# thomasdeppisch/eMagLS

Hardware: AMD Instinct MI355X
Metric: eMagLS filter sets/s (N=4, 2702 dirs, 512 taps) (higher is better)
Workload: dtype f64; 1 GPU; BASELINE config 3: getEMagLsFilters em32 r=4.2cm N=4 complex-SH, 2702 dirs, 512 taps, 48 kHz; one filter set per step, inputs resident in HBM; dirs=2702, taps=512, sim_order=19, bins=512, k_cut=43, designs_resident_per_gpu=128, designs_per_batch=32, batches_in_flight=4, distinct_hrir_sets_resident=20, parallelism=independent jobs per GPU, one RCCL gather

## Files before the change

### emagls_amd/build.py

```python
from __future__ import annotations

import argparse
import os
import subprocess
import sys
from concurrent.futures import ThreadPoolExecutor

HERE = os.path.dirname(os.path.abspath(__file__))
CSRC = os.path.join(HERE, "csrc")
OBJ = os.path.join(HERE, "build")
LIBDIR = os.path.join(HERE, "lib")
LIB = os.path.join(LIBDIR, "libemagls.so")
SOURCES = ["sh_basis.hip", "modal.hip", "fft.hip", "gram_chol.hip", "factor.hip", "gramroute.hip", "sweep.hip", "sweep_persist.hip", "sweep_synth.hip", "sweep_reg.hip", "synth_debug.hip", "factor_debug.hip", "fft_debug.hip", "gram_debug.hip", "dspace.hip", "atf.hip", "decode.hip", "decode_stream.hip", "field_stream.hip", "rotate.hip", "rotate3.hip", "resample.hip", "render.hip", "render_api.hip", "response.hip", "response_api.hip", "array_irs.hip", "shoebox.hip", "array_irs_api.hip", "emash.hip", "wide.hip", "wide_array.hip", "microbench.hip",
           "switches.hip", "decode_api.hip", "field_api.hip", "host_pools.hip", "plan_setup.hip", "plan_run.hip", "batch_run.hip", "capi.hip", "jobs.hip"]
HIPCC = os.environ.get("HIPCC", "/opt/rocm/bin/hipcc")
FLAGS = ["--offload-arch=gfx950", "-O3", "-std=c++17", "-fPIC", "-ffp-contract=off", "-Wall", "-Wno-unused-function",
         "-Wno-unused-result", "-Wno-unused-value"]


def _newest_header():
    hs = [os.path.join(CSRC, f) for f in os.listdir(CSRC) if f.endswith(".hpp")]
    hs.append(os.path.join(os.path.dirname(HERE), "include", "emagls.h"))
    return max(os.path.getmtime(h) for h in hs)


def _compile(src, force):
    obj = os.path.join(OBJ, src.replace(".hip", ".o"))
    srcp = os.path.join(CSRC, src)
# ... 38 lines not shown
```

### emagls_amd/csrc/batch_run.hip

```cpp
#include "host_internal.hpp"

void emagls_batch_forget(emagls_batch* b, emagls_plan* p) {
    for (auto& q : b->plans) if (q == p) q = nullptr;
}

namespace {
void batch_sweep_stage(emagls_batch& b) {
    const int nb = (int)b.plans.size();
    std::vector<HalfSweepArgs> ha((size_t)nb);
    for (int j = 0; j < nb; ++j) ha[j] = emagls_half_args(*b.plans[j]);
    if (b.atf_share || b.geo_share)
        for (int j = 1; j < nb; ++j) {
            ha[j].G = ha[0].G; ha[j].Yri = ha[0].Yri; ha[j].Mw = ha[0].Mw; ha[j].cond_ok = ha[0].cond_ok;
            ha[j].bsc = ha[0].bsc; ha[j].smap = ha[0].smap;
            ha[j].skip_flag = ha[0].skip_flag;
        }
    const bool reg = b.plans[0]->sweep_persist && reg_sweep_wanted(b.plans.data(), nb);
    for (auto* q : b.plans) q->reg_sweep = reg;
    if (!reg && nb > SWEEP_MULTI_MAX) throw Error(EMAGLS_ERR_UNSUPPORTED, "internal: more than 16 designs in a batch need the register-resident sweep");
    HalfSweepMulti h{};
    h.n = std::min(nb, SWEEP_MULTI_MAX);
    for (int j = 0; j < h.n; ++j) h.a[j] = ha[j];
    emagls_plan& q0 = *b.plans[0];
    const int kk0 = std::max(q0.kcut0, 1);
// ... 102 lines not shown
    HIP_CHECK(hipStreamSynchronize(b.stream));
    HIP_CHECK(hipMemsetAsync(b.cmp_flag.get(), 0, 16, b.stream));
    emagls_plan& p0 = *b.plans[0];
    for (size_t j = 1; j < b.plans.size(); ++j)
        for (const char* name : names) launch_compare_words(p0.get(name), b.plans[j]->get(name), p0.bufs[name].bytes, b.cmp_flag.get<int>(), b.stream);
    int differ = 0;
    HIP_CHECK(hipMemcpyAsync(&differ, b.cmp_flag.get(), sizeof differ, hipMemcpyDeviceToHost, b.stream));
    HIP_CHECK(hipStreamSynchronize(b.stream));
    checked_version = ver;
    return same = differ == 0;
}
void batch_set_sharing(emagls_batch& b, bool& field, bool share) {
    if (share == field) return;
    for (auto* p : b.plans) drop_plan_graphs(*p);
    drop_batch_graphs(b);
    if (&field == &b.geo_share) batch_geo_forget(b);
    field = share;
}
void batch_run_two_graphs(emagls_batch& b, CapturedGraph& pre, void (*stage)(emagls_batch&, int), int pre_part, int launches) {
    const bool replay = b.use_graph && b.eager_runs >= 1;
    if (replay && !pre) pre.capture(b.stream, [&] { stage(b, pre_part); });
    if (replay && !b.post) b.post.capture(b.stream, [&] { stage(b, 2); });
    b.used = 0;
    if (replay) pre.launch(b.stream); else stage(b, pre_part);
    batch_sweep_stage(b);
    if (replay) b.post.launch(b.stream); else stage(b, 2);
    mark_executed(b, launches);
    if (!replay) ++b.eager_runs;
}
template <typename Pre> void batch_run_per_plan(emagls_batch& b, bool replay, Pre pre, void (*post)(emagls_plan&), int launches) {
    emagls_plan& p0 = *b.plans[0];
// ... 52 lines not shown
    for (auto* p : b.plans)
        if (!p->have_hrirs || !p->have_hrir_grid || !p->have_atfs)
            throw Error(EMAGLS_ERR_ARG, "every plan of the batch needs its HRIRs, its grid and the ATFs");
    batch_atf_decide_sharing(b);
    emagls_plan& p0 = *b.plans[0];
    if (b.atf_share && p0.sweep_persist) { batch_run_two_graphs(b, b.group[0], batch_atf_shared_stage, 0, 1); return; }
    batch_run_per_plan(b, b.use_graph && b.eager_runs >= 1,
                       [&](emagls_plan& p) { if (b.atf_share && &p != &p0) from_atf_subject_pre_stage(p); else plan_pre_stage(p); },
                       from_atf_post_sweep, sweep_launch_count(p0));
}

uint64_t batch_geo_version(const emagls_batch& b) {
    uint64_t ver = 0;
    for (const emagls_plan* p : b.plans) ver = (ver * 1000003ull + p->atf_side_version) * 1000003ull + p->solo_runs;
    return ver;
}
void batch_geo_decide_sharing(emagls_batch& b) {
    bool share = false;
    if (b.geo_want && b.plans.size() > 1) {
        emagls_plan& p0 = *b.plans[0];
        bool eligible = (p0.d.kind == EMAGLS_KIND_EMAGLS || p0.d.kind == EMAGLS_KIND_EMAGLS2 || p0.d.kind == EMAGLS_KIND_EMA_CH) && !p0.wide &&
                        !p0.diffuse && !p0.custom_basis;
        for (auto* p : b.plans) {
            const emagls_design_desc &x = p->d, &y = p0.d;
            eligible = eligible && x.kind == y.kind && x.order == y.order && x.fs == y.fs && x.len == y.len && x.nsamp == y.nsamp &&
                       x.ndirs == y.ndirs && x.mic_radius == y.mic_radius && x.nmics == y.nmics && x.basis == y.basis &&
                       x.sim_order_pad == y.sim_order_pad && p->wide == p0.wide && p->diffuse == p0.diffuse && p->custom_basis == p0.custom_basis &&
                       p->real_internal == p0.real_internal && p->gram_from == p0.gram_from && p->hh_end == p0.hh_end && p->n_h == p0.n_h &&
                       p->g0 == p0.g0 && p->sweep_persist == p0.sweep_persist;
        }
        share = eligible && batch_inputs_same(b, {"hrir_azi", "hrir_zen", "mic_azi", "mic_zen"}, b.geo_checked_version, b.geo_inputs_same);
    }
    batch_set_sharing(b, b.geo_share, share);
}
void geo_hrir_side(emagls_plan& h, emagls_plan& g, emagls_plan& p0, hipStream_t st) {
    subject_reset(h, st);
    h.sync_used = 0;
    hrir_spectra(h, p0, st);
    if (g.hh_end > 1) {
        hrir_hh_rows(h, g, st);
        hrir_hh_back(hh_factor_args(h, g, nullptr, g.get<double>("cond_ok")), g, st);
    }
    hrir_gram_ls_rows(h, g, p0, true, st);
    if (p0.synth) launch_synth_winit(h.get("W"), p0.get("Pm"), p0.C, (int)p0.d.nmics, std::max(p0.kcut0, 1), p0.P, h.get("Winit"), st, true);
}
void batch_geo_stage(emagls_batch& b, int part) {
    emagls_plan& p0 = *b.plans[0];
    StreamLoan loan(b.plans, b.stream);
    const int n = (int)b.plans.size();
    auto hrir_side = [&](int first) {
        if (first >= n) return;
        if (b.lanes) {
            BatchScope sc(n - first, b.stride);
            geo_hrir_side(*b.plans[first], *b.plans[first], p0, b.stream);
        } else {
            for (int j = first; j < n; ++j) geo_hrir_side(*b.plans[j], p0, p0, b.stream);
        }
    };
    if (part == 1) {
        hrir_side(0);
    } else if (part == 0) {
        plan_pre_stage(p0);
        if (b.lanes && n > 1) {
            emagls_plan& g = p0;
            const bool cb = g.cplx_basis;
            const int gf = g.gram_from, hh_end = g.hh_end, ldSh = g.ldS_h;
            const int ls_end = std::min(g.kcut0, g.P);
            const size_t g_stride_b = sizeof(cplx) * (size_t)g.C * g.ldD;
            auto bc = [&](const char* name, size_t off, size_t bytes) {
                if (!g.has(name) || bytes == 0) return;
                bytes = std::min(bytes, g.bufs[name].bytes - off);
                launch_broadcast_lanes(g.get<char>(name) + off, bytes, b.stride, n - 1, b.stream);
            };
            if (hh_end > 1) {
                bc("Yc", 0, g.bufs["Yc"].bytes);
                bc(cb ? "R" : "Rc", 0, g.bufs[cb ? "R" : "Rc"].bytes);
                bc("Vws", 0, sizeof(cplx) * (size_t)(hh_end - 1) * g.C * ldSh);
                bc("Nw", 0, sizeof(cplx) * (size_t)(hh_end - 1) * g.C * g.C);
                bc("tauw", 0, sizeof(double) * (size_t)(hh_end - 1) * g.C);
                bc("cond_ok", 0, sizeof(double) * (size_t)g.P);
            }
            if (gf > 0 && gf < ls_end) {
                bc("G", (size_t)(gf - g.g0) * g_stride_b, (size_t)(ls_end - gf) * g_stride_b);
                bc("Mw", 0, sizeof(cplx) * (size_t)ls_end * g.C * g.C);
            }
        }
        hrir_side(1);
    } else if (b.lanes) {
        BatchScope sc(n, b.stride);
        Scoped from(p0.geo_from, &p0);
        emagls_post_sweep(p0);
    } else {
        for (auto* p : b.plans) {
            Scoped from(p->geo_from, &p0);
            emagls_post_sweep(*p);
        }
    }
}
void batch_execute_geo(emagls_batch& b) {
    const bool warm = batch_geo_next_is_warm(b);
    if (!warm) {
        b.geo_kept_version = ~0ull;
        b.geo_ran_version = batch_geo_version(b);
        b.geo_cold_pending = true;
    }
    batch_run_two_graphs(b, warm ? b.warm : b.group[0], batch_geo_stage, warm ? 1 : 0, sweep_launch_count(*b.plans[0]));
    b.last_form = warm ? 2 : 1;
    ++(warm ? b.geo_warm_runs : b.geo_cold_runs);
}

void batch_magls_decide_sharing(emagls_batch& b, bool sweep_needed) {
    bool share = false;
    emagls_plan& p0 = *b.plans[0];
    if (b.geo_want && b.plans.size() > 1 && !p0.custom_basis && !p0.diffuse && (p0.sweep_persist || !sweep_needed)) {
        share = batch_inputs_same(b, {"hrir_azi", "hrir_zen"}, b.geo_checked_version, b.geo_inputs_same);
        for (auto* p : b.plans) share = share && !p->custom_basis && p->d.fs == p0.d.fs;
    }
    batch_set_sharing(b, b.geo_share, share);
}
// ... 286 lines not shown
```

### emagls_amd/csrc/capi.hip

```cpp
#include "host_internal.hpp"

namespace {

struct CachedPlan {
    std::unique_ptr<emagls_plan> plan;
    emagls_design_desc desc{};
    int device = 0;
    bool busy = false;
    uint64_t last_use = 0;
};
std::mutex g_cache_mu;
std::vector<CachedPlan> g_cache;
uint64_t g_cache_tick = 0;

int one_shot(const emagls_design_desc& desc, const double* hL, const double* hR, const double* azi, const double* zen,
             const double* mic_azi, const double* mic_zen, const double* atf, const double* atf_azi, const double* atf_zen,
             void* wL, void* wR, double* mean_dev, const void* Y_hrir = nullptr, const void* Y_mic = nullptr) {
    return guarded([&] {
        int dev = 0;
        HIP_CHECK(hipGetDevice(&dev));
        emagls_plan* p = nullptr;
        std::unique_ptr<emagls_plan> fresh;
        bool cached = false;
        {
// ... 424 lines not shown
            for (int i = 0; i < p->sweep_launches && 2 * (size_t)i + 1 < p->sweep_events.size(); ++i) {
                float t = 0.f;
                HIP_CHECK(hipEventElapsedTime(&t, p->sweep_events[2 * i], p->sweep_events[2 * i + 1]));
                tot += t;
                ++n;
            }
        }
        *total_ms = tot;
        *launches = n;
    });
}
int emagls_plan_debug_buffer(emagls_plan* p, const char* name, void* dst, size_t* nbytes) {
    return guarded([&] {
        DeviceGuard dg(p ? p->device : -1);
        if (!p || !name || !nbytes) throw Error(EMAGLS_ERR_ARG, "null pointer");
        auto it = p->bufs.find(name);
        if (it == p->bufs.end()) throw Error(EMAGLS_ERR_ARG, std::string("unknown buffer ") + name);
        if (!dst) { *nbytes = it->second.bytes; return; }
        HIP_CHECK(hipStreamSynchronize(p->stream));
        const size_t n = std::min(*nbytes, it->second.bytes);
        HIP_CHECK(hipMemcpy(dst, it->second.p, n, hipMemcpyDeviceToHost));
        *nbytes = n;
    });
}
void* emagls_plan_stream(emagls_plan* p) { return p ? (void*)p->stream : nullptr; }

int emagls_batch_create(emagls_plan** plans, int nplans, emagls_batch** batch) {
    return guarded([&] {
        if (!plans || !batch || nplans < 1) throw Error(EMAGLS_ERR_ARG, "invalid argument");
        const int batch_max = std::max(g_batch_max.load(), g_batch_max_override);
// ... 387 lines not shown
```

### emagls_amd/csrc/dspace.hip

```cpp
#include "kernels.hpp"

namespace emagls {

constexpr double COND_LIMIT = 1.0e4;

template <typename T, int QT_TD>
__global__ void __launch_bounds__(512) qt_kernel(const T* __restrict__ Yc, int64_t ldY, const T* __restrict__ E, int ldE,
                                                 int D, int S, int C, int nOrders, T* __restrict__ QT, int64_t ldD, size_t bstride) {
    Yc = boff(Yc, bstride); E = boff(E, bstride); QT = boff(QT, bstride);
    extern __shared__ __attribute__((aligned(16))) char dyn[];
    T* ys = reinterpret_cast<T*>(dyn);
    const int ldq = S + 1;
    const int d0 = blockIdx.x * QT_TD;
    for (int idx = threadIdx.x; idx < QT_TD * S; idx += blockDim.x) {
        const int dl = idx / S, s = idx % S;
        ys[(size_t)dl * ldq + s] = (d0 + dl < D) ? Yc[(int64_t)(d0 + dl) * ldY + s] : zero_of<T>();
    }
    __syncthreads();
    const int dl = threadIdx.x % QT_TD;
    const T* y = ys + (size_t)dl * ldq;
    for (int c = threadIdx.x / QT_TD; c < C; c += 512 / QT_TD) {
        const T* e = E + (int64_t)c * ldE;
        for (int n = 0; n < nOrders; ++n) {
            const int sb = n * n, se = min(S, (n + 1) * (n + 1));
// ... 150 lines not shown
__global__ void cond_flag_kernel(const double* __restrict__ sv, int C, int P, int hh_end, double* __restrict__ cond_ok, size_t bstride) {
    sv = boff(sv, bstride); cond_ok = boff(cond_ok, bstride);
    const int kb = blockIdx.x * blockDim.x + threadIdx.x;
    if (kb >= P) return;
    double smax = 0.0, smin = INFINITY;
    for (int i = 0; i < C; ++i) { const double s = sv[(int64_t)kb * C + i]; smax = fmax(smax, s); smin = fmin(smin, s); }
    cond_ok[kb] = (kb >= hh_end || smax <= COND_LIMIT * smin) ? 1.0 : 0.0;
}

template <typename T>
__global__ void __launch_bounds__(256) yri_accurate_kernel(const T* __restrict__ Q, int64_t ldQ, const cplx* __restrict__ Z,
                                                           int ldS, const double* __restrict__ cond_ok, int D, int S, int C, int k0,
                                                           cplx* __restrict__ Yri, int64_t ldD, size_t bstride) {
    Q = boff(Q, bstride); Z = boff(Z, bstride); cond_ok = boff(cond_ok, bstride); Yri = boff(Yri, bstride);
    const int kb = k0 + blockIdx.y;
    if (cond_ok[kb] != 0.0) return;
    const int c = threadIdx.x >> 3, dl = threadIdx.x & 7;
    if (c >= C) return;
    for (int d = blockIdx.x * 8 + dl; d < D; d += gridDim.x * 8) {
        const T* q = Q + (int64_t)d * ldQ;
        const cplx* z = Z + ((int64_t)kb * C + c) * ldS;
        cplx a0 = mk(0, 0), a1 = mk(0, 0);
        int s = 0;
        for (; s + 1 < S; s += 2) { cfma(a0, conj(q[s]), z[s]); cfma(a1, conj(q[s + 1]), z[s + 1]); }
        if (s < S) cfma(a0, conj(q[s]), z[s]);
        Yri[((int64_t)(kb - k0) * C + c) * ldD + d] = a0 + a1;
    }
}

constexpr int YA_SCH = 32;
__global__ void __launch_bounds__(256) yri_accurate_cm_kernel(const double* __restrict__ Ycm, int64_t ldY, const cplx* __restrict__ Z, int ldS,
                                                              const double* __restrict__ cond_ok, int D, int S, int C, int k0,
                                                              cplx* __restrict__ Yri, int64_t ldD, size_t bstride) {
    Ycm = boff(Ycm, bstride); Z = boff(Z, bstride); cond_ok = boff(cond_ok, bstride); Yri = boff(Yri, bstride);
    const int kb = k0 + blockIdx.y;
    if (cond_ok[kb] != 0.0) return;
    __shared__ __attribute__((aligned(16))) cplx zs[32][YA_SCH + 1];
    const int tid = threadIdx.x, wave = tid >> 6, lane = tid & 63;
    const int d = blockIdx.x * 128 + (wave & 1) * 64 + lane;
    const int ch0 = (wave >> 1) * 16;
    const int dc = d < D ? d : D - 1;
    cplx acc[16];
#pragma unroll
    for (int i = 0; i < 16; ++i) acc[i] = mk(0, 0);
    for (int s0 = 0; s0 < S; s0 += YA_SCH) {
        __syncthreads();
        for (int idx = tid; idx < 32 * YA_SCH; idx += 256) {
            const int c = idx / YA_SCH, s = idx % YA_SCH;
            zs[c][s] = (c < C && s0 + s < S) ? Z[((int64_t)kb * C + c) * ldS + s0 + s] : mk(0, 0);
        }
        __syncthreads();
// ... 108 lines not shown
```

### emagls_amd/csrc/gram_chol.hip

```cpp
#include <cstdlib>
#include <vector>

#include "device_mem.hpp"

namespace emagls {

typedef double double4_t __attribute__((ext_vector_type(4)));
typedef double double2_t __attribute__((ext_vector_type(2)));

template <typename T> struct GramAcc;
template <> struct GramAcc<double> {
    double4_t r[2][2];
    __device__ void init() { for (int a = 0; a < 2; ++a) for (int b = 0; b < 2; ++b) r[a][b] = double4_t{0, 0, 0, 0}; }
};
template <> struct GramAcc<cplx> {
    double4_t r[2][2], i[2][2];
    __device__ void init() {
        for (int a = 0; a < 2; ++a) for (int b = 0; b < 2; ++b) { r[a][b] = double4_t{0, 0, 0, 0}; i[a][b] = double4_t{0, 0, 0, 0}; }
    }
};

__device__ __forceinline__ void gram_step(GramAcc<double>& acc, const double (&a)[2], const double (&b)[2]) {
#pragma unroll
    for (int x = 0; x < 2; ++x)
// ... 572 lines not shown
            KERNEL_CHECK();
            chol_update_kernel<T><<<bgrid(nbt * (nbt + 1) / 2), 256, 0, st>>>((T*)G, S, j0, nbt, batch_ctx().stride);
            KERNEL_CHECK();
        }
    }
}
void launch_cholesky(void* G, int S, bool is_cplx, int* flag, hipStream_t st) {
    if (is_cplx) chol_impl<cplx>(G, S, flag, st); else chol_impl<double>(G, S, flag, st);
}

__global__ void __launch_bounds__(256) zsolve_flagged_kernel(cplx* __restrict__ Z, int ldS, const cplx* __restrict__ R,
                                                             const cplx* __restrict__ Rinv, const double* __restrict__ cond_ok,
                                                             int S, int C, int k0, size_t bstride) {
    Z = boff(Z, bstride); R = boff(R, bstride); Rinv = boff(Rinv, bstride); cond_ok = boff(cond_ok, bstride);
    const int kb = k0 + blockIdx.x;
    if (cond_ok[kb] != 0.0) return;
    __shared__ cplx as[32][33];
    __shared__ cplx ri[32][33];
    const int c = threadIdx.x >> 3, part = threadIdx.x & 7;
    cplx* z = Z + ((int64_t)kb * C + (c < C ? c : 0)) * ldS;
    const int nblk = (S + NB - 1) / NB;
    for (int J = nblk - 1; J >= 0; --J) {
        const int j0 = J * NB;
        for (int idx = threadIdx.x; idx < NB * NB; idx += 256) ri[idx / NB][idx % NB] = Rinv[(int64_t)J * NB * NB + idx];
        for (int m = 0; m < 4; ++m) {
            const int jj = part + 8 * m, j = j0 + jj;
            cplx acc = mk(0, 0);
            if (c < C && j < S) {
                acc = z[j];
                const cplx* rrow = R + (int64_t)j * S;
                for (int i = j0 + NB; i < S; ++i) { cplx p = mk(0, 0); cfma(p, z[i], conj(rrow[i])); acc = acc - p; }
// ... 119 lines not shown
```

### emagls_amd/csrc/host_internal.hpp

```cpp
#pragma once
#include <atomic>
#include <chrono>
#include <cstdlib>
#include <cstring>
#include <deque>
#include <map>
#include <memory>
#include <mutex>
#include <shared_mutex>
#include <string>
#include <thread>
#include <utility>
#include <vector>

#include "../../include/emagls.h"
#include "array_model.hpp"
#include "device_mem.hpp"
#include "kernels.hpp"

using namespace emagls;

struct emagls_batch;
void emagls_batch_forget(emagls_batch* b, emagls_plan* p);

// ... 326 lines not shown
    bool lanes = false;
    size_t stride = 0;
    hipStream_t stream = nullptr;
    bool own_stream = true;
    bool atf = false, atf_share = false, atf_inputs_same = false;
    uint64_t atf_checked_version = ~0ull;
    bool magls = false;
    bool geo_want = false, geo_share = false, geo_inputs_same = false;
    uint64_t geo_checked_version = ~0ull;
    uint64_t geo_kept_version = ~0ull;
    uint64_t geo_ran_version = ~0ull;
    bool geo_cold_pending = false;
    CapturedGraph warm;
    int last_form = 0;
    long long geo_cold_runs = 0, geo_warm_runs = 0;
    emagls::DevMem cmp_flag;
    int nstreams = 1;
    hipStream_t side[3] = {nullptr, nullptr, nullptr};
    CapturedGraph group[4];
    int prof_level = 0;
    hipEvent_t sweep_ev[2] = {nullptr, nullptr};
    CapturedGraph post;
    bool side0_external = false;
    int order_hint = 0;
    int groups = 1;
    CapturedGraph group_hh[4];
    hipStream_t hh_stream[4] = {nullptr, nullptr, nullptr, nullptr};
    bool defer_hh = false;
    bool alone = true;
    int eager_runs = 0;
// ... 47 lines not shown

constexpr double GRAM_COND_EST = 3.0e3;

inline bool forks_streams(const emagls_plan& p) { return p.nstreams >= 2; }

extern thread_local hipStream_t g_plan_stream_shared;
void plan_routes(emagls_plan& p);
void synth_pairing(const double* azi, const double* zen, int M, int* smap);
void plan_alloc_routes(emagls_plan& p);
void plan_setup(emagls_plan& p);

void stage_prologue(emagls_plan& p, int mode, const int64_t* didx, int64_t Dh);
void execute_ls(emagls_plan& p);
void magls_post_sweep(emagls_plan& p);
bool plan_defers_hh_route(const emagls_plan& p);
void hrir_spectra(emagls_plan& h, const emagls_plan& g, hipStream_t st);
FactorArgs hh_factor_args(emagls_plan& h, emagls_plan& g, int* sweeps_out, double* cond_ok);
void hrir_hh_rows(emagls_plan& h, emagls_plan& g, hipStream_t st);
void hrir_hh_back(const FactorArgs& fa, const emagls_plan& g, hipStream_t st);
void hrir_gram_ls_rows(emagls_plan& h, emagls_plan& g, const emagls_plan& src, bool lanes_share, hipStream_t st);
void subject_reset(emagls_plan& p, hipStream_t st);
void emagls_pre_sweep(emagls_plan& p);
HalfSweepArgs emagls_half_args(emagls_plan& p);
struct SweepGate {
    struct Entry { hipEvent_t ev; int slots; };
    struct State { std::deque<Entry> inflight; std::vector<hipEvent_t> pool; int capacity = 0; };
    static std::mutex& mutex();
    static State& state();
    std::unique_lock<std::mutex> lock;
    hipStream_t st;
    int slots;
// ... 30 lines not shown
```

### emagls_amd/csrc/kernels.hpp

```cpp
#pragma once
#include <algorithm>
#include <functional>

#include "common.hpp"

namespace emagls {

void launch_zero(void* p, size_t bytes, hipStream_t st);
void launch_compare_words(const void* a, const void* b, size_t bytes, int* differ, hipStream_t st);
void launch_broadcast_lanes(const void* src, size_t bytes, size_t stride, int nlanes, hipStream_t st);
struct LanePtrs { void* p[64]; };
void launch_scatter_lanes(const void* srcL, const void* srcR, size_t stride, size_t bytes, int n, const LanePtrs& dst, hipStream_t st);
void launch_gather_buffers(const LanePtrs& src, const LanePtrs& dst, int nbuf, size_t bytes, hipStream_t st);
struct BufferMoves { const void* src[96]; void* dst[96]; size_t bytes[96]; int n; };
void launch_move_buffers(const BufferMoves& m, hipStream_t st);
void launch_ch_basis(int N, int M, const double* azi, bool cplx_basis, void* out, int ld, hipStream_t st, bool out_real = false);
void launch_sh_coeff(int N, double* tab, hipStream_t st);
inline size_t esz(bool c) { return c ? sizeof(cplx) : sizeof(double); }
inline size_t sh_coeff_count(int N) { return (size_t)2 * (N + 1) * (N + 1) + 2 * (N + 1); }
void launch_sh_basis(int N, int64_t D, const double* azi, const double* zen, const double* tab, bool cplx_basis,
                     void* Y, int64_t ld, hipStream_t st);
void launch_transpose_conj(const void* Y, int64_t D, int64_t S, int64_t ldY, void* Yt, int64_t Dpad, int64_t ldYt,
                           bool is_cplx, bool conj_it, hipStream_t st);

// ... 65 lines not shown
int persist_sweep_dpw(int D);
int sweep_cu_budget();
bool persist_sweep_fits(int D, int C, int ndesigns);
bool synth_sweep_fits(int D, int nmics, int nOrd, int ndesigns);
bool synth_sweep_supported(int D, int nmics, int nOrd);
int synth_nord_pad(int nOrd);
void launch_synth_prepare(const void* bn, int nOrd, int P, void* bsc, const void* Zlo, int ldZ, int nOut, int M, const int* smap, double* Pm, hipStream_t st);
void launch_synth_mt(const void* Mw, const double* Pm, int nOut, int M, int k0, int P, const void* W, void* Mt, void* Winit, hipStream_t st);
void launch_synth_winit(const void* W, const void* Pm, int nOut, int M, int k0, int P, void* Winit, hipStream_t st, bool shared_geometry);
void launch_synth_rows(const void* U, int nchunks, const void* Pm, const void* Mw, int nOut, int M, int k_lo, int k_hi, int P, void* W, hipStream_t st,
                       bool shared_geometry = false);
int synth_ls_chunks(int D);
void launch_synth_ls(const void* Hc, int64_t ldH, int n_c, const void* bsc, int nord_pad, const double* dir_azi, const double* dir_zen, const double* mic_azi,
                     const double* mic_zen, const int* smap, int D, int M, int P, int kb_lo, int kb_hi, void* Upart, hipStream_t st, bool shared_geometry = false);
void launch_sweep_synth(const HalfSweepMulti& m, hipStream_t st);
void synth_cosines_debug(const double* dir_azi, const double* dir_zen, int64_t ndirs, const double* mic_azi, const double* mic_zen, int nmics, double* x2);
void synth_operand_debug(const void* bsc, int nbins, int nord_pad, const double* x, int64_t nx, int gs, void* g_plus, void* g_minus);
int reg_sweep_max_units();
bool reg_sweep_supported(int D, int nmics, int nunits, int nOrd);
size_t reg_sweep_ll_bytes(int D, int nmics);
int reg_sweep_capacity(int D);
int reg_sweep_slots_per_xcd();
int reg_sweep_pick_waves(int D, int ndesigns);
int reg_sweep_gate_cost(int D, int ndesigns);
bool reg_sweep_fits(int D, int nmics, int nunits, int nOrd, int ndesigns);
void launch_sweep_reg(const HalfSweepArgs* args_dev, const HalfSweepArgs& a0, int n, hipStream_t st);
double reg_contract_selftest();
double gram_tile_selftest(bool four);
void store_sweep_args(const HalfSweepArgs* host, int n, HalfSweepArgs* dev, hipStream_t st);
void launch_sweep_finalize(const void* Wpart, void* W, int nWG, int C, int P, int kb_last, hipStream_t st);
// ... 205 lines not shown
```

### emagls_amd/csrc/plan_run.hip

```cpp
#include "host_internal.hpp"

namespace {
void stage_hrir_basis(emagls_plan& p) {
    hipStream_t st = p.stream;
    const bool cb = p.cplx_basis;
    if (p.d.kind == EMAGLS_KIND_MAGLS_2D) {
        launch_ch_basis(p.d.order, (int)p.D, p.get<double>("hrir_azi"), cb, p.get("Ycm"), (int)p.ldD, st, !cb);
    } else if (!p.custom_basis) {
        launch_sh_coeff(p.simOrder, p.get<double>("sh_tab"), st);
        launch_sh_basis(p.simOrder, p.D, p.get<double>("hrir_azi"), p.get<double>("hrir_zen"), p.get<double>("sh_tab"), cb,
                        p.get("Ycm"), p.ldD, st);
    }
    launch_transpose_conj(p.get("Ycm"), p.D, p.S, p.ldD, p.get("Yc"), p.Dpad, p.ldS, cb, true, st);
    p.mark("sh_basis");
    launch_gram(p.get("Yc"), p.D, p.S, p.ldS, cb, p.get("Gp"), nullptr, p.get("R"), p.S, st);
    p.mark("gram_mfma");
    launch_cholesky(p.get("R"), p.S, cb, p.get<int>("flag"), st);
    p.mark("cholesky");
    if (p.wide) return;
    launch_qform(p.get("Yc"), p.get("R"), p.get("Rinv"), p.S, p.D, p.ldS, cb, p.get("Q"), st);
    p.mark("qform");
}

void record_sweep_event(emagls_plan& p, size_t i) {
// ... 487 lines not shown
void magls_post_sweep(emagls_plan& p) {
    hipStream_t st = p.stream;
    const bool cb = p.cplx_basis;
    if (p.diffuse)
        launch_diffuse_constraint(p.get("W"), p.get("Xc"), cb, 0, 1, p.get("Hfull"), (int)p.D, p.C, p.ldD, p.P, st);
    launch_filter_epilogue(p.get("W"), p.C, p.nfft, (int)p.d.len, p.get("tw"), p.get<double>("grpd"),
                           cb ? (p.d.kind == EMAGLS_KIND_MAGLS_2D ? 2 : 1) : 0, 0, 0,
                           p.out_cplx ? 1 : 0, p.get("wL"), p.get("wR"), st);
    p.mark("epilogue");
}

bool plan_defers_hh_route(const emagls_plan& p) {
    const int k0 = std::max(p.kcut0, 1);
    return sw_int<Sw::DEFER_HH>() != 0 && p.synth && !p.diffuse && p.prof_level == 0 && p.d.kind != EMAGLS_KIND_EMA_SH && p.gram_from > 0 && p.hh_end > 1 && p.hh_end <= k0 - 1;
}
void hrir_spectra(emagls_plan& h, const emagls_plan& g, hipStream_t st) {
    const emagls_design_desc& d = h.d;
    const int ls_end = std::min(g.kcut0, g.P);
    launch_twiddles(h.nfft, h.get("tw"), st);
    launch_hrir_grpdelay(h.get<double>("hL"), h.get<double>("hR"), d.nsamp, d.ndirs, h.nfft, h.get("tw"), h.get<double>("dirsum"),
                         h.get<double>("grpd"), st);
    launch_hrir_fft(h.get<double>("hL"), h.get<double>("hR"), d.nsamp, h.D, nullptr, h.nfft, h.get("tw"), h.get<double>("grpd"), 0, ls_end,
                    h.kcut0, h.get("Hc"), h.get<double>("Habs"), h.ldD, st, ls_end > 0 ? h.get<double>("HcT") : nullptr,
                    round_up(4 * std::max(ls_end, 1), 64));
}
FactorArgs hh_factor_args(emagls_plan& h, emagls_plan& g, int* sweeps_out, double* cond_ok) {
    const int ls_end = std::min(g.kcut0, g.P);
    FactorArgs fa{};
    fa.S = g.S_h; fa.C = g.C; fa.ldS = g.ldS_h; fa.kb0 = 1; fa.P = g.P;
    fa.Tn = g.get("Tn"); fa.bn = g.get<cplx>("bn"); fa.nOrders = g.n_h + 1; fa.bn_stride = g.simOrder + 1;
    fa.reg_mode = 0; fa.reg_c = SVD_REGUL_CONST;
    fa.Z = h.get<cplx>("Z");
    fa.Mw = g.get<cplx>("Mw");
    fa.Vws = g.get<cplx>("Vws"); fa.sv = g.get<double>("sv");
    fa.Hq = h.get<cplx>("Hq"); fa.ldHq = g.ldS_h; fa.hq_estride = (int64_t)ls_end * g.ldS_h; fa.ls_end = std::min(ls_end, g.hh_end);
    fa.hq_conj = 1;
    fa.route = g.get<int>("route"); fa.status = h.get<int>("flag");
    fa.cond_limit = 10.0 * GRAM_COND_EST;
// ... 453 lines not shown
```

### emagls_amd/csrc/switches.hpp

```cpp
#pragma once
#include <climits>
#include <cmath>

namespace emagls {

#define EMAGLS_SWITCHES(X) \
    X(PLAN_CACHE,        INT,  4,     0, INT_MAX,   PROCESS, "shapes the one-shot entry points keep alive (0 = off)") \
    X(BATCH_MAX,         INT,  8,     1, 32,        PROCESS, "initial limit of designs per batch, read at load time (emagls_set_batch_max changes it at run time; the job scheduler sets it per chunk)") \
    X(BATCH_GROUPS,      INT,  2,     1, 4,         CALL,    "lane groups of a batch of more than 8 designs before its sweep (1 = one launch sequence)") \
    X(BATCH_LANES,       ON0,  1,     0, 1,         CALL,    "=0: batches in stream mode (per-plan pipelines) instead of lane mode") \
    X(DEBUG_LANES,       ON1,  0,     0, 1,         CALL,    "=1: why a batch was refused lane mode or common routes, on stderr") \
    X(STAGGER,           ON0,  1,     0, 1,         PROCESS, "=0: both lane groups of a batch issue the stages before the sweep in one order (default: complementary orders)") \
    X(DEFER_HH,          INT,  1,     0, 2,         PROCESS, "the orthonormal route of the low bins next to the sweep: 0 never, 1 batches and designs that have the device to themselves, 2 every lane batch") \
    X(GEO_KEEP,          ON0,  1,     0, 1,         PROCESS, "=0: sharing batches run their geometry stages on every execute") \
    X(GRAM_LDS,          ON0,  1,     0, 1,         PROCESS, "=0: lane batches take the K-split Gram kernel + reduce instead of the LDS-staged one") \
    X(GRAM_MFMA4,        ON1,  0,     0, 1,         CALL,    "=1: the Gram tile on the 4 x 4 x 4 MFMA shape (measured slower; the tests' second form)") \
    X(XCD_RUNS,          ON0,  1,     0, 1,         PROCESS, "=0: gram_lds, gemm_tn_f64, synth_ls take their tiles in dispatch order instead of XCD-aware runs") \
    X(GRAM_ROUTE,        ON0,  1,     0, 1,         CALL,    "=0: no Gram route (all bins Householder + Jacobi)") \
    X(GRAM_COND_EST,     REAL, 3e3,   -HUGE_VAL, HUGE_VAL, CALL, "conditioning estimate below which the Gram route starts (the device check stays at 3e4)") \
    X(JACOBI_RUN,        INT,  0,     1, INT_MAX,   PROCESS, "bins per Jacobi workgroup on the Gram route (0: single bins where the stages are forked, runs of 2 in lane groups)") \
    X(REAL_INTERNAL,     ON0,  1,     0, 1,         CALL,    "=0: complex-basis eMagLS / eMagLS2 designs on the complex-arithmetic pipeline") \
    X(NO_GRAPH,          ON1,  0,     0, 1,         CALL,    "=1: eager launches instead of hipGraph replay (plans and batches, when they are created)") \
    X(STREAMS,           INT,  0,     1, 4,         CALL,    "streams of a single plan (0: one, until emagls_plan_set_streams)") \
    X(ONESHOT_STREAMS,   INT,  1,     1, 3,         CALL,    "streams of the one-shot plans of array designs") \
    X(SWEEP_PERSIST,     ON0,  1,     0, 1,         CALL,    "=0: launch-per-bin sweep instead of the persistent one") \
    X(PERSIST_GLOBAL,    ON1,  0,     0, 1,         CALL,    "=1: write-through granules even when a design sits on one XCD") \
    X(SWEEP_SYNTH,       ON0,  1,     0, 1,         CALL,    "=0: array designs on materialised operands instead of the synthesising sweep (when a plan is created)") \
    X(SWEEP_TWIN,        ON0,  1,     0, 1,         CALL,    "=0: launches of 9-16 designs as two independent workgroups per CU instead of twin workgroups") \
    X(SWEEP_REG,         INT,  1,     0, 2,         CALL,    "register-resident sweep: 0 never (the slab form), 1 for launches of more than 8 designs, 2 always") \
// ... 56 lines not shown
```

Measured before the change: 3919 filter sets/s.

## Share one least-squares operand per bin across geometry-sharing HRIR batches

When every plan in a batch shares the array and HRIR geometry, the per-bin Y_reg_inv least-squares operand is computed once for the batch. That covers the Householder/Z-solve bins and the Gram bins through a new synthesis kernel. Each HRIR set then needs only its spectra plus a small Hc·Yls row product kernel, instead of carrying its own LS rows through the factor chain. The batch keeps extra device buffers and invalidates its graphs whenever they reallocate. It also adds a switch, on by default, to turn the path off.

After: 4309 filter sets/s, median of 6. 1.1x the previous value.

```diff
diff --git a/emagls_amd/build.py b/emagls_amd/build.py
--- a/emagls_amd/build.py
+++ b/emagls_amd/build.py
@@ -11,7 +11,7 @@
 OBJ = os.path.join(HERE, "build")
 LIBDIR = os.path.join(HERE, "lib")
 LIB = os.path.join(LIBDIR, "libemagls.so")
-SOURCES = ["sh_basis.hip", "modal.hip", "fft.hip", "gram_chol.hip", "factor.hip", "gramroute.hip", "sweep.hip", "sweep_persist.hip", "sweep_synth.hip", "sweep_reg.hip", "synth_debug.hip", "factor_debug.hip", "fft_debug.hip", "gram_debug.hip", "dspace.hip", "atf.hip", "decode.hip", "decode_stream.hip", "field_stream.hip", "rotate.hip", "rotate3.hip", "resample.hip", "render.hip", "render_api.hip", "response.hip", "response_api.hip", "array_irs.hip", "shoebox.hip", "array_irs_api.hip", "emash.hip", "wide.hip", "wide_array.hip", "microbench.hip",
+SOURCES = ["sh_basis.hip", "modal.hip", "fft.hip", "gram_chol.hip", "factor.hip", "gramroute.hip", "sweep.hip", "sweep_persist.hip", "sweep_synth.hip", "sweep_reg.hip", "ls_shared.hip", "synth_debug.hip", "factor_debug.hip", "fft_debug.hip", "gram_debug.hip", "dspace.hip", "atf.hip", "decode.hip", "decode_stream.hip", "field_stream.hip", "rotate.hip", "rotate3.hip", "resample.hip", "render.hip", "render_api.hip", "response.hip", "response_api.hip", "array_irs.hip", "shoebox.hip", "array_irs_api.hip", "emash.hip", "wide.hip", "wide_array.hip", "microbench.hip",
            "switches.hip", "decode_api.hip", "field_api.hip", "host_pools.hip", "plan_setup.hip", "plan_run.hip", "batch_run.hip", "capi.hip", "jobs.hip"]
 HIPCC = os.environ.get("HIPCC", "/opt/rocm/bin/hipcc")
 FLAGS = ["--offload-arch=gfx950", "-O3", "-std=c++17", "-fPIC", "-ffp-contract=off", "-Wall", "-Wno-unused-function",
diff --git a/emagls_amd/csrc/batch_run.hip b/emagls_amd/csrc/batch_run.hip
--- a/emagls_amd/csrc/batch_run.hip
+++ b/emagls_amd/csrc/batch_run.hip
@@ -140,7 +140,7 @@
     if (share == field) return;
     for (auto* p : b.plans) drop_plan_graphs(*p);
     drop_batch_graphs(b);
-    if (&field == &b.geo_share) batch_geo_forget(b);
+    if (&field == &b.geo_share || &field == &b.geo_ls_shared) batch_geo_forget(b);
     field = share;
 }
 void batch_run_two_graphs(emagls_batch& b, CapturedGraph& pre, void (*stage)(emagls_batch&, int), int pre_part, int launches) {
@@ -223,6 +223,12 @@
     uint64_t ver = 0;
     for (const emagls_plan* p : b.plans) ver = (ver * 1000003ull + p->atf_side_version) * 1000003ull + p->solo_runs;
     return ver;
+}
+static bool batch_geo_ls_shared_wanted(const emagls_plan& p0) {
+    const int ls_end = std::min(p0.kcut0, p0.P);
+    const bool gram_ls = p0.gram_from > 0 && p0.gram_from < ls_end;
+    return sw_on<Sw::GEO_LS_SHARED>() && p0.d.kind != EMAGLS_KIND_EMAGLS2 && ls_end > 1 && p0.C <= 32 && (!gram_ls || p0.synth) &&
+           (p0.hh_end <= 1 || p0.has("Z"));
 }
 void batch_geo_decide_sharing(emagls_batch& b) {
     bool share = false;
@@ -241,6 +247,7 @@
         share = eligible && batch_inputs_same(b, {"hrir_azi", "hrir_zen", "mic_azi", "mic_zen"}, b.geo_checked_version, b.geo_inputs_same);
     }
     batch_set_sharing(b, b.geo_share, share);
+    batch_set_sharing(b, b.geo_ls_shared, share && batch_geo_ls_shared_wanted(*b.plans[0]));
 }
 void geo_hrir_side(emagls_plan& h, emagls_plan& g, emagls_plan& p0, hipStream_t st) {
     subject_reset(h, st);
@@ -253,17 +260,50 @@
     hrir_gram_ls_rows(h, g, p0, true, st);
     if (p0.synth) launch_synth_winit(h.get("W"), p0.get("Pm"), p0.C, (int)p0.d.nmics, std::max(p0.kcut0, 1), p0.P, h.get("Winit"), st, true);
 }
+void geo_spectra_side(emagls_plan& h, emagls_plan& p0, hipStream_t st) {
+    subject_reset(h, st);
+    h.sync_used = 0;
+    hrir_spectra(h, p0, st, false);
+}
+void geo_ls_shared_rows(emagls_plan& h, emagls_plan& p0, const void* yls, hipStream_t st) {
+    launch_ls_shared_rows(h.get("Hc"), h.ldD, std::min(p0.kcut0, p0.P), yls, p0.ldD, (int)p0.D, p0.C, p0.P, h.get("W"), st);
+    if (p0.synth) launch_synth_winit(h.get("W"), p0.get("Pm"), p0.C, (int)p0.d.nmics, std::max(p0.kcut0, 1), p0.P, h.get("Winit"), st, true);
+}
+void geo_yls_stage(emagls_batch& b, hipStream_t st) {
+    emagls_plan& g = *b.plans[0];
+    const bool cb = g.cplx_basis;
+    const int ls_end = std::min(g.kcut0, g.P), hh_ls = std::min(g.hh_end, ls_end), gf = g.gram_from;
+    cplx* yls = b.yls.get<cplx>();
+    if (hh_ls > 1) {
+        HIP_CHECK(hipMemcpyAsync(b.zls.get(), g.get("Z"), sizeof(cplx) * (size_t)hh_ls * g.C * g.ldS_h, hipMemcpyDeviceToDevice, st));
+        launch_zsolve_flagged(b.zls.get(), g.ldS_h, g.get(cb ? "R" : "Rc"), g.get(cb ? "Rinv" : "Rinvc"), nullptr, g.S_h, g.C, hh_ls, 1, st);
+        launch_yri_accurate(g.get("Yc"), g.ldS, cb, b.zls.get(), g.ldS_h, nullptr, (int)g.D, g.S_h, g.C, hh_ls, 1, yls, g.ldD, st,
+                            g.custom_basis ? nullptr : g.get("Ycm"), g.ldD);
+    }
+    if (gf > 0 && gf < ls_end)
+        launch_yls_gram(g.get("bsc"), synth_nord_pad(g.simOrder + 1), g.get<double>("hrir_azi"), g.get<double>("hrir_zen"), g.get<double>("mic_azi"),
+                        g.get<double>("mic_zen"), g.get<int>("smap"), g.get<double>("Pm"), g.get("Mw"), (int)g.D, g.C, gf, ls_end,
+                        yls, g.ldD, st);
+}
 void batch_geo_stage(emagls_batch& b, int part) {
     emagls_plan& p0 = *b.plans[0];
     StreamLoan loan(b.plans, b.stream);
     const int n = (int)b.plans.size();
-    auto hrir_side = [&](int first) {
+    auto each = [&](int first, auto f) {
         if (first >= n) return;
         if (b.lanes) {
             BatchScope sc(n - first, b.stride);
-            geo_hrir_side(*b.plans[first], *b.plans[first], p0, b.stream);
+            f(*b.plans[first], *b.plans[first]);
         } else {
-            for (int j = first; j < n; ++j) geo_hrir_side(*b.plans[j], p0, p0, b.stream);
+            for (int j = first; j < n; ++j) f(*b.plans[j], p0);
+        }
+    };
+    auto hrir_side = [&](int first) {
+        if (b.geo_ls_shared) {
+            each(first, [&](emagls_plan& h, emagls_plan&) { geo_spectra_side(h, p0, b.stream); });
+            each(0, [&](emagls_plan& h, emagls_plan&) { geo_ls_shared_rows(h, p0, b.yls.get(), b.stream); });
+        } else {
+            each(first, [&](emagls_plan& h, emagls_plan& g) { geo_hrir_side(h, g, p0, b.stream); });
         }
     };
     if (part == 1) {
@@ -294,6 +334,7 @@
                 bc("Mw", 0, sizeof(cplx) * (size_t)ls_end * g.C * g.C);
             }
         }
+        if (b.geo_ls_shared) geo_yls_stage(b, b.stream);
         hrir_side(1);
     } else if (b.lanes) {
         BatchScope sc(n, b.stride);
@@ -312,6 +353,14 @@
         b.geo_kept_version = ~0ull;
         b.geo_ran_version = batch_geo_version(b);
         b.geo_cold_pending = true;
+        if (b.geo_ls_shared) {
+            const emagls_plan& p0 = *b.plans[0];
+            const int ls_end = std::min(p0.kcut0, p0.P), hh_ls = std::min(p0.hh_end, ls_end);
+            const void *y0 = b.yls.get(), *z0 = b.zls.get();
+            b.yls.grow(sizeof(cplx) * (size_t)(ls_end - 1) * p0.C * p0.ldD);
+            b.zls.grow(sizeof(cplx) * (size_t)std::max(hh_ls, 1) * p0.C * p0.ldS_h);
+            if (b.yls.get() != y0 || b.zls.get() != z0) { b.group[0].reset(); b.warm.reset(); }
+        }
     }
     batch_run_two_graphs(b, warm ? b.warm : b.group[0], batch_geo_stage, warm ? 1 : 0, sweep_launch_count(*b.plans[0]));
     b.last_form = warm ? 2 : 1;
diff --git a/emagls_amd/csrc/capi.hip b/emagls_amd/csrc/capi.hip
--- a/emagls_amd/csrc/capi.hip
+++ b/emagls_amd/csrc/capi.hip
@@ -462,6 +462,18 @@
     return guarded([&] {
         DeviceGuard dg(p ? p->device : -1);
         if (!p || !name || !nbytes) throw Error(EMAGLS_ERR_ARG, "null pointer");
+        if (std::string(name) == "Yls") {
+            emagls_batch* b = p->owner;
+            if (!b || !b->geo_share || !b->geo_ls_shared || !b->yls.get()) throw Error(EMAGLS_ERR_ARG, "Yls: the plan's batch keeps no such operand");
+            const emagls_plan& p0 = *b->plans[0];
+            const size_t bytes = sizeof(cplx) * (size_t)(std::min(p0.kcut0, p0.P) - 1) * p0.C * p0.ldD;
+            if (!dst) { *nbytes = bytes; return; }
+            HIP_CHECK(hipStreamSynchronize(b->stream));
+            const size_t n = std::min(*nbytes, bytes);
+            HIP_CHECK(hipMemcpy(dst, b->yls.get(), n, hipMemcpyDeviceToHost));
+            *nbytes = n;
+            return;
+        }
         auto it = p->bufs.find(name);
         if (it == p->bufs.end()) throw Error(EMAGLS_ERR_ARG, std::string("unknown buffer ") + name);
         if (!dst) { *nbytes = it->second.bytes; return; }
diff --git a/emagls_amd/csrc/dspace.hip b/emagls_amd/csrc/dspace.hip
--- a/emagls_amd/csrc/dspace.hip
+++ b/emagls_amd/csrc/dspace.hip
@@ -188,7 +188,7 @@
                                                            cplx* __restrict__ Yri, int64_t ldD, size_t bstride) {
     Q = boff(Q, bstride); Z = boff(Z, bstride); cond_ok = boff(cond_ok, bstride); Yri = boff(Yri, bstride);
     const int kb = k0 + blockIdx.y;
-    if (cond_ok[kb] != 0.0) return;
+    if (cond_ok && cond_ok[kb] != 0.0) return;
     const int c = threadIdx.x >> 3, dl = threadIdx.x & 7;
     if (c >= C) return;
     for (int d = blockIdx.x * 8 + dl; d < D; d += gridDim.x * 8) {
@@ -208,7 +208,7 @@
                                                               cplx* __restrict__ Yri, int64_t ldD, size_t bstride) {
     Ycm = boff(Ycm, bstride); Z = boff(Z, bstride); cond_ok = boff(cond_ok, bstride); Yri = boff(Yri, bstride);
     const int kb = k0 + blockIdx.y;
-    if (cond_ok[kb] != 0.0) return;
+    if (cond_ok && cond_ok[kb] != 0.0) return;
     __shared__ __attribute__((aligned(16))) cplx zs[32][YA_SCH + 1];
     const int tid = threadIdx.x, wave = tid >> 6, lane = tid & 63;
     const int d = blockIdx.x * 128 + (wave & 1) * 64 + lane;
diff --git a/emagls_amd/csrc/gram_chol.hip b/emagls_amd/csrc/gram_chol.hip
--- a/emagls_amd/csrc/gram_chol.hip
+++ b/emagls_amd/csrc/gram_chol.hip
@@ -610,7 +610,7 @@
                                                              int S, int C, int k0, size_t bstride) {
     Z = boff(Z, bstride); R = boff(R, bstride); Rinv = boff(Rinv, bstride); cond_ok = boff(cond_ok, bstride);
     const int kb = k0 + blockIdx.x;
-    if (cond_ok[kb] != 0.0) return;
+    if (cond_ok && cond_ok[kb] != 0.0) return;
     __shared__ cplx as[32][33];
     __shared__ cplx ri[32][33];
     const int c = threadIdx.x >> 3, part = threadIdx.x & 7;
diff --git a/emagls_amd/csrc/host_internal.hpp b/emagls_amd/csrc/host_internal.hpp
--- a/emagls_amd/csrc/host_internal.hpp
+++ b/emagls_amd/csrc/host_internal.hpp
@@ -364,6 +364,8 @@
     CapturedGraph warm;
     int last_form = 0;
     long long geo_cold_runs = 0, geo_warm_runs = 0;
+    bool geo_ls_shared = false;
+    emagls::DevMem yls, zls;
     emagls::DevMem cmp_flag;
     int nstreams = 1;
     hipStream_t side[3] = {nullptr, nullptr, nullptr};
@@ -441,7 +443,7 @@
 void execute_ls(emagls_plan& p);
 void magls_post_sweep(emagls_plan& p);
 bool plan_defers_hh_route(const emagls_plan& p);
-void hrir_spectra(emagls_plan& h, const emagls_plan& g, hipStream_t st);
+void hrir_spectra(emagls_plan& h, const emagls_plan& g, hipStream_t st, bool transposed = true);
 FactorArgs hh_factor_args(emagls_plan& h, emagls_plan& g, int* sweeps_out, double* cond_ok);
 void hrir_hh_rows(emagls_plan& h, emagls_plan& g, hipStream_t st);
 void hrir_hh_back(const FactorArgs& fa, const emagls_plan& g, hipStream_t st);
diff --git a/emagls_amd/csrc/kernels.hpp b/emagls_amd/csrc/kernels.hpp
--- a/emagls_amd/csrc/kernels.hpp
+++ b/emagls_amd/csrc/kernels.hpp
@@ -103,6 +103,9 @@
 void launch_synth_ls(const void* Hc, int64_t ldH, int n_c, const void* bsc, int nord_pad, const double* dir_azi, const double* dir_zen, const double* mic_azi,
                      const double* mic_zen, const int* smap, int D, int M, int P, int kb_lo, int kb_hi, void* Upart, hipStream_t st, bool shared_geometry = false);
 void launch_sweep_synth(const HalfSweepMulti& m, hipStream_t st);
+void launch_yls_gram(const void* bsc, int nord_pad, const double* dir_azi, const double* dir_zen, const double* mic_azi, const double* mic_zen,
+                     const int* smap, const double* Pm, const void* Mw, int D, int nOut, int kb_lo, int kb_hi, void* Yls, int64_t ldD, hipStream_t st);
+void launch_ls_shared_rows(const void* Hc, int64_t ldH, int ls_end, const void* Yls, int64_t ldD, int D, int C, int P, void* W, hipStream_t st);
 void synth_cosines_debug(const double* dir_azi, const double* dir_zen, int64_t ndirs, const double* mic_azi, const double* mic_zen, int nmics, double* x2);
 void synth_operand_debug(const void* bsc, int nbins, int nord_pad, const double* x, int64_t nx, int gs, void* g_plus, void* g_minus);
 int reg_sweep_max_units();
diff --git a/emagls_amd/csrc/ls_shared.hip b/emagls_amd/csrc/ls_shared.hip
--- /dev/null
+++ b/emagls_amd/csrc/ls_shared.hip
@@ -0,0 +1,145 @@
+#include "kernels.hpp"
+#include "persist_common.hpp"
+#include "synth_common.hpp"
+
+namespace emagls {
+
+namespace {
+
+__global__ void __launch_bounds__(256) yls_gram_kernel(const cplx* __restrict__ bsc, int nord_pad, const double* __restrict__ dir_azi,
+                                                       const double* __restrict__ dir_zen, const double* __restrict__ mic_azi,
+                                                       const double* __restrict__ mic_zen, const int* __restrict__ smap, const double* __restrict__ Pm,
+                                                       const cplx* __restrict__ Mw, int D, int nOut, int kb_lo, cplx* __restrict__ Yls, int64_t ldD) {
+    __shared__ __attribute__((aligned(16))) cplx bs[SY_NORD];
+    __shared__ double pm[PS_CMAX][PS_CMAX + 1];
+    __shared__ cplx mks[PS_CMAX * PS_CMAX];
+    const int tid = threadIdx.x, kb = kb_lo + (int)blockIdx.y;
+    const int npr = smap[32], nsg = smap[33];
+    if (tid < nord_pad) bs[tid] = bsc[(int64_t)kb * nord_pad + tid];
+    for (int idx = tid; idx < PS_CMAX * PS_CMAX; idx += 256) {
+        const int c = idx / PS_CMAX, j = idx % PS_CMAX;
+        pm[c][j] = c < nOut ? Pm[c * PS_CMAX + j] : 0.0;
+    }
+    const cplx* Mk = Mw + (int64_t)(kb - 1) * nOut * nOut;
+    for (int idx = tid; idx < nOut * nOut; idx += 256) mks[idx] = conj(Mk[idx]);
+    __syncthreads();
+    const int d = (int)blockIdx.x * 256 + tid, dc = d < D ? d : D - 1;
+    double sd, cd;
+    synth_zen(dir_zen[dc], sd, cd);
+    const double daz = dir_azi[dc];
+    cplx t[PS_CMAX];
+#pragma unroll
+    for (int c = 0; c < PS_CMAX; ++c) t[c] = mk(0, 0);
+    for (int u = 0; u < npr + nsg; ++u) {
+        const bool paired = u < npr;
+        const int row = paired ? 2 * u : 2 * npr + (u - npr);
+        const int jm = smap[row];
+        double sm, cm;
+        synth_zen(mic_zen[jm], sm, cm);
+        double x2[1];
+        x2[0] = synth_x2(sd, cd, sm, cm, daz - mic_azi[jm]);
+        cplx accE[1], accO[1];
+        synth_group<1>(x2, accE, accO, bs, nord_pad);
+        const cplx gA = conj(accE[0] + accO[0]), gB = conj(accE[0] - accO[0]);
+#pragma unroll
+        for (int c = 0; c < PS_CMAX; ++c) cfma(t[c], gA, pm[c][row]);
+        if (paired) {
+#pragma unroll
+            for (int c = 0; c < PS_CMAX; ++c) cfma(t[c], gB, pm[c][row + 1]);
+        }
+    }
+    if (d >= D) return;
+    for (int c = 0; c < nOut; ++c) {
+        cplx y = mk(0, 0);
+#pragma unroll
+        for (int cp = 0; cp < PS_CMAX; ++cp)
+            if (cp < nOut) cfma(y, t[cp], mks[cp * nOut + c]);
+        Yls[((int64_t)(kb - 1) * nOut + c) * ldD + d] = y;
+    }
+}
+
+constexpr int LR_NT = 512, LR_ROWS = 16, LR_DT = 64, LR_NS = LR_NT / 32, LR_DPT = LR_DT / LR_NS, LR_YLD = LR_DT + 1;
+__global__ void __launch_bounds__(LR_NT) ls_rows_kernel(const cplx* __restrict__ Hc, int64_t ldH, int n_c, const cplx* __restrict__ Yls, int64_t ldD,
+                                                        int D, int C, int P, cplx* __restrict__ W, int nlanes, size_t bstride) {
+    __shared__ __attribute__((aligned(16))) cplx ys[32 * LR_YLD];
+    __shared__ __attribute__((aligned(16))) cplx hs[LR_ROWS * LR_DT];
+    static_assert(LR_NS * 4 * 32 <= 32 * LR_YLD, "the slices' sums of four rows fit the tile buffer");
+    const int tid = threadIdx.x, kb = 1 + (int)blockIdx.x, lane0 = (int)blockIdx.y * (LR_ROWS / 2);
+    const int c = tid & 31, ds = tid >> 5;
+    const int lrow = tid >> 6, lcol = tid & 63;
+    const cplx* Yk = Yls + (int64_t)(kb - 1) * C * ldD;
+    const cplx* hrow[2];
+    bool hok[2];
+#pragma unroll
+    for (int q = 0; q < 2; ++q) {
+        const int r = q * 8 + lrow, lane = lane0 + (r >> 1);
+        hok[q] = lane < nlanes;
+        hrow[q] = boffz(Hc, bstride, hok[q] ? (unsigned)lane : 0u) + ((int64_t)(r & 1) * n_c + kb) * ldH;
+    }
+    cplx yr[4], hr[2];
+    auto load = [&](int d0) __attribute__((always_inline)) {
+        const int d = d0 + lcol;
+#pragma unroll
+        for (int q = 0; q < 4; ++q) {
+            const int row = q * 8 + lrow;
+            yr[q] = (row < C && d < D) ? Yk[(int64_t)row * ldD + d] : mk(0, 0);
+        }
+#pragma unroll
+        for (int q = 0; q < 2; ++q) hr[q] = (hok[q] && d < D) ? hrow[q][d] : mk(0, 0);
+    };
+    cplx acc[LR_ROWS];
+#pragma unroll
+    for (int r = 0; r < LR_ROWS; ++r) acc[r] = mk(0, 0);
+    load(0);
+    for (int d0 = 0; d0 < D; d0 += LR_DT) {
+        __syncthreads();
+#pragma unroll
+        for (int q = 0; q < 4; ++q) ys[(q * 8 + lrow) * LR_YLD + lcol] = yr[q];
+#pragma unroll
+        for (int q = 0; q < 2; ++q) hs[(q * 8 + lrow) * LR_DT + lcol] = hr[q];
+        __syncthreads();
+        if (d0 + LR_DT < D) load(d0 + LR_DT);
+#pragma unroll
+        for (int i = 0; i < LR_DPT; ++i) {
+            const int dl = ds * LR_DPT + i;
+            const cplx y = ys[c * LR_YLD + dl];
+#pragma unroll
+            for (int r = 0; r < LR_ROWS; ++r) cfma(acc[r], hs[r * LR_DT + dl], y);
+        }
+    }
+    cplx* red = ys;
+#pragma unroll
+    for (int part = 0; part < LR_ROWS / 4; ++part) {
+        __syncthreads();
+#pragma unroll
+        for (int rr = 0; rr < 4; ++rr) red[(ds * 4 + rr) * 32 + c] = acc[part * 4 + rr];
+        __syncthreads();
+        if (tid < 4 * 32) {
+            const int rr = tid >> 5, r = part * 4 + rr, lane = lane0 + (r >> 1), e = r & 1;
+            cplx w = mk(0, 0);
+            for (int s = 0; s < LR_NS; ++s) w += red[(s * 4 + rr) * 32 + c];
+            if (c < C && lane < nlanes) boffz(W, bstride, (unsigned)lane)[((int64_t)e * P + kb) * C + c] = w;
+        }
+    }
+}
+
+}
+
+void launch_yls_gram(const void* bsc, int nord_pad, const double* dir_azi, const double* dir_zen, const double* mic_azi, const double* mic_zen,
+                     const int* smap, const double* Pm, const void* Mw, int D, int nOut, int kb_lo, int kb_hi, void* Yls, int64_t ldD, hipStream_t st) {
+    if (kb_hi <= kb_lo) return;
+    if (nOut > PS_CMAX || nord_pad > SY_NORD) throw Error(2, "ls_shared: more than 32 channels or 95 orders");
+    yls_gram_kernel<<<dim3((unsigned)ceil_div(D, 256), (unsigned)(kb_hi - kb_lo)), 256, 0, st>>>((const cplx*)bsc, nord_pad, dir_azi, dir_zen, mic_azi, mic_zen, smap, Pm,
+                                                                                               (const cplx*)Mw, D, nOut, kb_lo, (cplx*)Yls, ldD);
+    KERNEL_CHECK();
+}
+void launch_ls_shared_rows(const void* Hc, int64_t ldH, int ls_end, const void* Yls, int64_t ldD, int D, int C, int P, void* W, hipStream_t st) {
+    if (ls_end <= 1) return;
+    if (C > 32) throw Error(2, "ls_shared: more than 32 channels");
+    const int nlanes = batch_ctx().n;
+    ls_rows_kernel<<<dim3((unsigned)(ls_end - 1), (unsigned)ceil_div(2 * nlanes, LR_ROWS)), LR_NT, 0, st>>>((const cplx*)Hc, ldH, ls_end, (const cplx*)Yls, ldD, D, C, P,
+                                                                                                          (cplx*)W, nlanes, batch_ctx().stride);
+    KERNEL_CHECK();
+}
+
+}
diff --git a/emagls_amd/csrc/plan_run.hip b/emagls_amd/csrc/plan_run.hip
--- a/emagls_amd/csrc/plan_run.hip
+++ b/emagls_amd/csrc/plan_run.hip
@@ -525,14 +525,14 @@
     const int k0 = std::max(p.kcut0, 1);
     return sw_int<Sw::DEFER_HH>() != 0 && p.synth && !p.diffuse && p.prof_level == 0 && p.d.kind != EMAGLS_KIND_EMA_SH && p.gram_from > 0 && p.hh_end > 1 && p.hh_end <= k0 - 1;
 }
-void hrir_spectra(emagls_plan& h, const emagls_plan& g, hipStream_t st) {
+void hrir_spectra(emagls_plan& h, const emagls_plan& g, hipStream_t st, bool transposed) {
     const emagls_design_desc& d = h.d;
     const int ls_end = std::min(g.kcut0, g.P);
     launch_twiddles(h.nfft, h.get("tw"), st);
     launch_hrir_grpdelay(h.get<double>("hL"), h.get<double>("hR"), d.nsamp, d.ndirs, h.nfft, h.get("tw"), h.get<double>("dirsum"),
                          h.get<double>("grpd"), st);
     launch_hrir_fft(h.get<double>("hL"), h.get<double>("hR"), d.nsamp, h.D, nullptr, h.nfft, h.get("tw"), h.get<double>("grpd"), 0, ls_end,
-                    h.kcut0, h.get("Hc"), h.get<double>("Habs"), h.ldD, st, ls_end > 0 ? h.get<double>("HcT") : nullptr,
+                    h.kcut0, h.get("Hc"), h.get<double>("Habs"), h.ldD, st, (transposed && ls_end > 0) ? h.get<double>("HcT") : nullptr,
                     round_up(4 * std::max(ls_end, 1), 64));
 }
 FactorArgs hh_factor_args(emagls_plan& h, emagls_plan& g, int* sweeps_out, double* cond_ok) {
diff --git a/emagls_amd/csrc/switches.hpp b/emagls_amd/csrc/switches.hpp
--- a/emagls_amd/csrc/switches.hpp
+++ b/emagls_amd/csrc/switches.hpp
@@ -13,6 +13,7 @@
     X(STAGGER,           ON0,  1,     0, 1,         PROCESS, "=0: both lane groups of a batch issue the stages before the sweep in one order (default: complementary orders)") \
     X(DEFER_HH,          INT,  1,     0, 2,         PROCESS, "the orthonormal route of the low bins next to the sweep: 0 never, 1 batches and designs that have the device to themselves, 2 every lane batch") \
     X(GEO_KEEP,          ON0,  1,     0, 1,         PROCESS, "=0: sharing batches run their geometry stages on every execute") \
+    X(GEO_LS_SHARED,     ON0,  1,     0, 1,         CALL,    "=0: sharing batches carry every HRIR set's least-squares rows through the factors instead of one kept Y_reg_inv per bin") \
     X(GRAM_LDS,          ON0,  1,     0, 1,         PROCESS, "=0: lane batches take the K-split Gram kernel + reduce instead of the LDS-staged one") \
     X(GRAM_MFMA4,        ON1,  0,     0, 1,         CALL,    "=1: the Gram tile on the 4 x 4 x 4 MFMA shape (measured slower; the tests' second form)") \
     X(XCD_RUNS,          ON0,  1,     0, 1,         PROCESS, "=0: gram_lds, gemm_tn_f64, synth_ls take their tiles in dispatch order instead of XCD-aware runs") \
```
